# ubc-vision/COTR

Measured on NVIDIA H100. Metric: query-points/sec (256x256 pair, 1024 queries), higher is better.
Workload: dtype f32 (fp16 hi/lo split operands, fp32 accumulate on wgmma)

## Files before the change

### cotr_b200/csrc/mlp_tc.cu

```cuda
#include "split16.cuh"
#include "tc_common.cuh"

namespace cotr {

namespace {

using namespace tc;

constexpr int BM = 64;
constexpr int BK = 64;
constexpr int kThreads = 384;
constexpr int kConsumerThreads = 256;
constexpr int kBarConsumers = 6;
constexpr int kK1Chunks = kDModel / BK;

template <int S>
struct MlpCfg {
    static constexpr int HS = kFF / S;
    static constexpr int WN1 = HS / 2;
    static constexpr int kMain1 = WN1 >= 128 ? 1 : 2;
    static constexpr int kK2Chunks = HS / BK;
    static constexpr int kIters = kK1Chunks + kK2Chunks;
    static constexpr uint32_t kAPlane = BM * 128u;
    static constexpr uint32_t kW1Plane = HS * 128u;
    static constexpr uint32_t kW2Plane = kDModel * 128u;
    static constexpr uint32_t kStage1 = 2 * kAPlane + 2 * kW1Plane;
    static constexpr uint32_t kStage2 = 2 * kW2Plane;
    static constexpr uint32_t kStage = kStage1 > kStage2 ? kStage1 : kStage2;
    static constexpr uint32_t kHChunk = 2 * kAPlane;
    static constexpr uint32_t kHBytes = kK2Chunks * kHChunk;
    static constexpr int kStages = (int)((227u * 1024u - 2048u - kHBytes) / kStage);
    static constexpr uint32_t kHOffset = kStages * kStage;
    static constexpr uint32_t kBarOffset = kHOffset + kHBytes;
    static constexpr uint32_t kSmemBytes = kBarOffset + 256 + 1024;
    static constexpr uint32_t kAccPitch = kDModel * 4u + 16u;
    static constexpr uint32_t kAccBytes = ((BM * kAccPitch + 1023u) / 1024u) * 1024u;
    static constexpr int kOwnRows = BM / S;
    static constexpr uint32_t kRowBytes = kDModel * 4u;
    static constexpr uint32_t kPartOffset = kAccBytes;
    static constexpr uint32_t kPartBytes = (S - 1) * kOwnRows * kRowBytes;
    static_assert(kStages >= 2, "pipeline needs at least two stages");
    static_assert(kSmemBytes <= 227u * 1024u, "shared memory");
    static_assert(kPartOffset + kPartBytes <= kStages * kStage, "partial tiles do not fit the idle stages");
    static_assert(kStage % 1024 == 0 && kW1Plane % 1024 == 0 && kHBytes % 1024 == 0, "SWIZZLE_128B needs 1024-byte alignment");
};

template <int S>
__global__ void __launch_bounds__(kThreads, 1) mlp_tc_kernel(const MlpParams p) {
    using C = MlpCfg<S>;
    extern __shared__ uint8_t smem_raw[];
    const uint32_t raw_addr = smem_u32(smem_raw);
    uint8_t* base = smem_raw + (((raw_addr + 1023u) & ~1023u) - raw_addr);
    uint8_t* h_tile = base + C::kHOffset;
    uint64_t* full = reinterpret_cast<uint64_t*>(base + C::kBarOffset);
    uint64_t* empty = full + C::kStages;
    uint64_t* part_full = full + 2 * C::kStages;

    const int warp = threadIdx.x >> 5, lane = threadIdx.x & 31;
    const int rank = blockIdx.z;
    const int m0 = blockIdx.x * BM;
    const int h0 = rank * C::HS;

    if (threadIdx.x == 0) {
        for (int s = 0; s < C::kStages; ++s) {
            mbar_init(&full[s], 129);
            mbar_init(&empty[s], 8);
        }
        mbar_init(part_full, 1);
        mbar_fence_init();
        mbar_arrive_expect_tx(part_full, C::kPartBytes);
    }
    __syncthreads();

    if (warp >= 8) {
        const int t = threadIdx.x - kConsumerThreads;
        const int kg = t & 7;
        const int rb = t >> 3;
        const uint8_t* w1 = reinterpret_cast<const uint8_t*>(p.w1);
        const uint8_t* w2 = reinterpret_cast<const uint8_t*>(p.w2);
        auto load_weights = [&](int it) {
            const int s = it % C::kStages;
            uint8_t* dst = base + (size_t)s * C::kStage;
            if (it < kK1Chunks) {
                mbar_arrive_expect_tx(&full[s], 2u * C::kW1Plane);
                const uint8_t* src = w1 + ((size_t)(it * 2) * kFF + h0) * 128;
                tma_bulk_g2s(dst + 2 * C::kAPlane, src, C::kW1Plane, &full[s]);
                tma_bulk_g2s(dst + 2 * C::kAPlane + C::kW1Plane, src + (size_t)kFF * 128, C::kW1Plane, &full[s]);
            } else {
                mbar_arrive_expect_tx(&full[s], C::kStage2);
                tma_bulk_g2s(dst, w2 + (size_t)(h0 / BK + it - kK1Chunks) * C::kStage2, C::kStage2, &full[s]);
            }
        };
        if (t == 0) {
            for (int it = 0; it < C::kStages; ++it) load_weights(it);
            pdl_launch_dependents();
        }
        pdl_wait();
        const uint32_t a_off = (uint32_t)rb * 128u + (uint32_t)((kg ^ (rb & 7)) << 4);
#pragma unroll 1
        for (int it = 0; it < C::kIters; ++it) {
            const int s = it % C::kStages;
            const uint32_t ph = (uint32_t)(it / C::kStages) & 1u;
            mbar_wait(&empty[s], ph ^ 1u);
            if (t == 0 && it >= C::kStages) load_weights(it);
            if (it < kK1Chunks) {
                const uint32_t dst = smem_u32(base + (size_t)s * C::kStage) + a_off;
                const int k = it * BK + kg * 8;
#pragma unroll
                for (int i = 0; i < BM / 16; ++i) {
                    const int row = m0 + rb + 16 * i;
                    const bool ok = row < p.M;
                    const size_t off = ok ? (size_t)row * kDModel + k : 0;
                    cp_async16(dst + i * 2048, p.x.hi + off, ok ? 16u : 0u);
                    cp_async16(dst + C::kAPlane + i * 2048, p.x.lo + off, ok ? 16u : 0u);
                }
                cp_async_mbar_arrive_noinc(&full[s]);
            } else {
                mbar_arrive(&full[s]);
            }
        }
    } else {
        const int wg = warp >> 2;
        const int fr = (warp & 3) * 16 + (lane >> 2);
        const int fc = 2 * (lane & 3);
        {
            constexpr int WN = C::WN1, R = WN / 2;
            float acc_m[C::kMain1][R], acc_c[R];
#pragma unroll
            for (int a = 0; a < C::kMain1; ++a)
#pragma unroll
                for (int j = 0; j < R; ++j) acc_m[a][j] = 0.f;
#pragma unroll
            for (int j = 0; j < R; ++j) acc_c[j] = 0.f;
            auto mma = [&](float (&d)[R], uint64_t da, uint64_t db) {
                if constexpr (WN == 64) wgmma_ss_n64(d, da, db);
                else wgmma_ss_n128(d, da, db);
            };
            auto fence_all = [&]() {
#pragma unroll
                for (int a = 0; a < C::kMain1; ++a) fence_regs(acc_m[a]);
                fence_regs(acc_c);
            };
#pragma unroll 1
            for (int it = 0; it < kK1Chunks; ++it) {
                const int s = it % C::kStages;
                mbar_wait(&full[s], (uint32_t)(it / C::kStages) & 1u);
                fence_proxy_async_smem();
                const uint32_t a_addr = smem_u32(base + (size_t)s * C::kStage);
                const uint32_t b_addr = a_addr + 2 * C::kAPlane + (uint32_t)wg * WN * 128u;
                fence_all();
                wgmma_fence();
#pragma unroll
                for (int ks = 0; ks < BK / 16; ++ks) {
                    const uint64_t dah = make_desc_sw128(a_addr + 32 * ks);
                    const uint64_t dal = make_desc_sw128(a_addr + C::kAPlane + 32 * ks);
                    const uint64_t dbh = make_desc_sw128(b_addr + 32 * ks);
                    const uint64_t dbl = make_desc_sw128(b_addr + C::kW1Plane + 32 * ks);
                    mma(acc_c, dal, dbh);
                    mma(acc_m[ks % C::kMain1], dah, dbh);
                    mma(acc_c, dah, dbl);
                }
                wgmma_commit();
                wgmma_wait<1>();
                fence_all();
                if (it > 0 && lane == 0) mbar_arrive(&empty[(it - 1) % C::kStages]);
            }
            wgmma_wait<0>();
            fence_all();
            if (lane == 0) mbar_arrive(&empty[(kK1Chunks - 1) % C::kStages]);
#pragma unroll
            for (int j = 0; j < R; j += 2) {
                const int row = fr + ((j >> 1) & 1) * 8;
                const int c = wg * WN + (j >> 2) * 8 + fc;
                float v[2];
#pragma unroll
                for (int e = 0; e < 2; ++e) {
                    float y = acc_m[0][j + e];
#pragma unroll
                    for (int a = 1; a < C::kMain1; ++a) y += acc_m[a][j + e];
                    v[e] = fmaxf((acc_c[j + e] + y) * p.w1_scale + __ldg(p.b1 + h0 + c + e), 0.f);
                }
                uint32_t hi, lo;
                split_f16x2(v[0], v[1], hi, lo);
                const int cc = c & 63;
                uint8_t* d = h_tile + (uint32_t)(c >> 6) * C::kHChunk + (uint32_t)row * 128u + (uint32_t)((((cc >> 3) ^ (row & 7)) << 4) + (cc & 7) * 2);
                *reinterpret_cast<uint32_t*>(d) = hi;
                *reinterpret_cast<uint32_t*>(d + C::kAPlane) = lo;
            }
            fence_proxy_async_smem();
            named_barrier_sync(kBarConsumers, kConsumerThreads);
        }
        {
            float acc_m[64], acc_c[64];
#pragma unroll
            for (int j = 0; j < 64; ++j) { acc_m[j] = 0.f; acc_c[j] = 0.f; }
#pragma unroll 1
            for (int it = kK1Chunks; it < C::kIters; ++it) {
                const int s = it % C::kStages;
                mbar_wait(&full[s], (uint32_t)(it / C::kStages) & 1u);
                const uint32_t a_addr = smem_u32(h_tile) + (uint32_t)(it - kK1Chunks) * C::kHChunk;
                const uint32_t b_addr = smem_u32(base + (size_t)s * C::kStage) + (uint32_t)wg * 128u * 128u;
                fence_regs(acc_m);
                fence_regs(acc_c);
                wgmma_fence();
#pragma unroll
                for (int ks = 0; ks < BK / 16; ++ks) {
                    const uint64_t dah = make_desc_sw128(a_addr + 32 * ks);
                    const uint64_t dal = make_desc_sw128(a_addr + C::kAPlane + 32 * ks);
                    const uint64_t dbh = make_desc_sw128(b_addr + 32 * ks);
                    const uint64_t dbl = make_desc_sw128(b_addr + C::kW2Plane + 32 * ks);
                    wgmma_ss_n128(acc_c, dal, dbh);
                    wgmma_ss_n128(acc_m, dah, dbh);
                    wgmma_ss_n128(acc_c, dah, dbl);
                }
                wgmma_commit();
                wgmma_wait<1>();
                fence_regs(acc_m);
                fence_regs(acc_c);
                if (it > kK1Chunks && lane == 0) mbar_arrive(&empty[(it - 1) % C::kStages]);
            }
            wgmma_wait<0>();
            fence_regs(acc_m);
            fence_regs(acc_c);
            named_barrier_sync(kBarConsumers, kConsumerThreads);
#pragma unroll
            for (int j = 0; j < 64; j += 2) {
                const int row = fr + ((j >> 1) & 1) * 8;
                const int col = wg * 128 + (j >> 2) * 8 + fc;
                *reinterpret_cast<float2*>(base + (uint32_t)row * C::kAccPitch + col * 4) =
                    make_float2(acc_c[j] + acc_m[j], acc_c[j + 1] + acc_m[j + 1]);
            }
        }
    }

    __syncthreads();
    cluster_arrive();
    cluster_wait();
    {
        const uint32_t part_local = smem_u32(base) + C::kPartOffset;
        constexpr int kPieces = (BM - C::kOwnRows) * (C::kRowBytes / 16);
#pragma unroll 1
        for (int i = threadIdx.x; i < kPieces; i += kThreads) {
            const int pr = i / (C::kRowBytes / 16), piece = i % (C::kRowBytes / 16);
            const int r = pr < rank * C::kOwnRows ? pr : pr + C::kOwnRows;
            const int q = r / C::kOwnRows;
            const uint32_t slot = (uint32_t)(rank < q ? rank : rank - 1);
            const float4 v = *reinterpret_cast<const float4*>(base + (uint32_t)r * C::kAccPitch + piece * 16);
            const uint32_t dst = part_local + (slot * C::kOwnRows + (uint32_t)(r % C::kOwnRows)) * C::kRowBytes + piece * 16;
            st_async_f32x4(map_to_cta(dst, (uint32_t)q), v.x, v.y, v.z, v.w, map_to_cta(smem_u32(part_full), (uint32_t)q));
        }
    }
    if (warp < C::kOwnRows) mbar_wait(part_full, 0);
#pragma unroll 1
    for (int w = warp; w < C::kOwnRows; w += kThreads / 32) {
        const int rr = rank * C::kOwnRows + w;
        const int row = m0 + rr;
        if (row < p.M) {
            pdl_wait();
            float v[8];
            const uint8_t* own = base + (uint32_t)rr * C::kAccPitch + lane * 32;
            const float4 a0 = *reinterpret_cast<const float4*>(own), a1 = *reinterpret_cast<const float4*>(own + 16);
            v[0] = a0.x; v[1] = a0.y; v[2] = a0.z; v[3] = a0.w; v[4] = a1.x; v[5] = a1.y; v[6] = a1.z; v[7] = a1.w;
#pragma unroll 1
            for (int slot = 0; slot < S - 1; ++slot) {
                const uint8_t* pp = base + C::kPartOffset + (uint32_t)(slot * C::kOwnRows + w) * C::kRowBytes + lane * 32;
                const float4 b0 = *reinterpret_cast<const float4*>(pp), b1 = *reinterpret_cast<const float4*>(pp + 16);
                v[0] += b0.x; v[1] += b0.y; v[2] += b0.z; v[3] += b0.w; v[4] += b1.x; v[5] += b1.y; v[6] += b1.z; v[7] += b1.w;
            }
            float bias[8], res[8];
            load_vec8(p.b2, lane, bias);
            const size_t off = (size_t)row * kDModel + lane * 8;
            load8_split(p.x, off, res);
#pragma unroll
            for (int j = 0; j < 8; ++j) v[j] = v[j] * p.w2_scale + bias[j] + res[j];
            warp_layernorm256(v, p.g, p.be, lane);
            if (p.g2) warp_layernorm256(v, p.g2, p.be2, lane);
            store8_split(p.out, off, v);
        }
    }
}

template <int S>
int configure(size_t* smem) {
    static unsigned long long configured = 0;
    *smem = MlpCfg<S>::kSmemBytes;
    if (first_use_on_device(&configured))
        COTR_CHECK_CUDA(cudaFuncSetAttribute(mlp_tc_kernel<S>, cudaFuncAttributeMaxDynamicSharedMemorySize, (int)MlpCfg<S>::kSmemBytes));
    return 0;
}

int max_clusters_of_8(int* out) {
    static int cached[64] = {0};
    int dev = 0;
    cudaGetDevice(&dev);
    if (cached[dev & 63] > 0) { *out = cached[dev & 63]; return 0; }
    size_t smem = 0;
    if (configure<8>(&smem)) return 1;
    cudaLaunchConfig_t cfg = {};
    cfg.gridDim = dim3(1, 1, 8);
    cfg.blockDim = dim3(kThreads);
    cfg.dynamicSmemBytes = smem;
    cudaLaunchAttribute attr[1];
    attr[0].id = cudaLaunchAttributeClusterDimension;
    attr[0].val.clusterDim.x = 1;
    attr[0].val.clusterDim.y = 1;
    attr[0].val.clusterDim.z = 8;
    cfg.attrs = attr;
    cfg.numAttrs = 1;
    int n = 0;
    COTR_CHECK_CUDA(cudaOccupancyMaxActiveClusters(&n, mlp_tc_kernel<8>, &cfg));
    cached[dev & 63] = n;
    *out = n;
    return 0;
}

template <int S>
int launch_split(const MlpParams& p, cudaStream_t s) {
    size_t smem = 0;
    if (configure<S>(&smem)) return 1;
    const dim3 grid((p.M + BM - 1) / BM, 1, S);
    COTR_CHECK_CUDA(launch_kernel_cluster(mlp_tc_kernel<S>, grid, dim3(kThreads), smem, s, S, p));
    return 0;
}

}

int launch_mlp_tc(const MlpParams& p, cudaStream_t s) {
    COTR_CHECK(p.M > 0 && p.w1 && p.w2 && p.b1 && p.b2 && p.g && p.be && (p.g2 == nullptr) == (p.be2 == nullptr),
               "mlp_tc: bad parameters (M %d)", p.M);
    const int tiles = (p.M + BM - 1) / BM;
    int n8 = 0;
    if (max_clusters_of_8(&n8)) return 1;
    return launch_mlp_tc_split(p, tiles <= n8 ? 8 : 4, s);
}

int launch_mlp_tc_split(const MlpParams& p, int S, cudaStream_t s) {
    COTR_CHECK(S == 4 || S == 8, "mlp_tc: hidden split %d (4 or 8)", S);
    return S == 8 ? launch_split<8>(p, s) : launch_split<4>(p, s);
}

}
```

### cotr_b200/csrc/tc_common.cuh

```cuda
#pragma once
#include <cuda_fp16.h>
#include <cuda_runtime.h>
#include <cstdint>

namespace cotr {
namespace tc {

__device__ __forceinline__ uint32_t smem_u32(const void* p) {
    return static_cast<uint32_t>(__cvta_generic_to_shared(p));
}

__device__ __forceinline__ void mbar_init(uint64_t* bar, uint32_t count) {
    asm volatile("mbarrier.init.shared::cta.b64 [%0], %1;" ::"r"(smem_u32(bar)), "r"(count) : "memory");
}
__device__ __forceinline__ void mbar_fence_init() {
    asm volatile("fence.mbarrier_init.release.cluster;" ::: "memory");
}
__device__ __forceinline__ void mbar_arrive(uint64_t* bar) {
    asm volatile("mbarrier.arrive.shared::cta.b64 _, [%0];" ::"r"(smem_u32(bar)) : "memory");
}
__device__ __forceinline__ void mbar_arrive_expect_tx(uint64_t* bar, uint32_t bytes) {
    asm volatile("mbarrier.arrive.expect_tx.shared::cta.b64 _, [%0], %1;" ::"r"(smem_u32(bar)), "r"(bytes) : "memory");
}
__device__ __forceinline__ bool mbar_try_wait(uint64_t* bar, uint32_t parity) {
    uint32_t ok;
    asm volatile(
        "{\n\t.reg .pred p;\n\t"
        "mbarrier.try_wait.parity.shared::cta.b64 p, [%1], %2;\n\t"
        "selp.u32 %0, 1, 0, p;\n\t}"
        : "=r"(ok)
        : "r"(smem_u32(bar)), "r"(parity)
        : "memory");
    return ok != 0;
}
__device__ __forceinline__ void mbar_wait(uint64_t* bar, uint32_t parity) {
    while (!mbar_try_wait(bar, parity)) {
    }
}

__device__ __forceinline__ void fence_proxy_async_smem() {
    asm volatile("fence.proxy.async.shared::cta;" ::: "memory");
}

__device__ __forceinline__ void ld_cg_32b(const void* p, uint4& a, uint4& b) {
    a = __ldcg(reinterpret_cast<const uint4*>(p));
    b = __ldcg(reinterpret_cast<const uint4*>(p) + 1);
}

__device__ __forceinline__ void cp_async16(uint32_t smem_dst, const void* gmem_src, uint32_t src_bytes) {
    asm volatile("cp.async.cg.shared.global [%0], [%1], 16, %2;" ::"r"(smem_dst), "l"(gmem_src), "r"(src_bytes) : "memory");
}
__device__ __forceinline__ void cp_async_mbar_arrive_noinc(uint64_t* bar) {
    asm volatile("cp.async.mbarrier.arrive.noinc.shared::cta.b64 [%0];" ::"r"(smem_u32(bar)) : "memory");
}

__device__ __forceinline__ void named_barrier_sync(int id, int threads) {
    asm volatile("bar.sync %0, %1;" ::"r"(id), "r"(threads) : "memory");
}

__device__ __forceinline__ void named_barrier_arrive(int id, int threads) {
    asm volatile("bar.arrive %0, %1;" ::"r"(id), "r"(threads) : "memory");
}

__device__ __forceinline__ void cluster_arrive() { asm volatile("barrier.cluster.arrive.release;" ::: "memory"); }
__device__ __forceinline__ void cluster_wait() { asm volatile("barrier.cluster.wait.acquire;" ::: "memory"); }
__device__ __forceinline__ uint32_t map_to_cta(uint32_t smem_addr, uint32_t rank) {
    uint32_t r;
    asm volatile("mapa.shared::cluster.u32 %0, %1, %2;" : "=r"(r) : "r"(smem_addr), "r"(rank));
    return r;
}
__device__ __forceinline__ void st_cluster_f32x4(uint32_t cluster_addr, float a, float b, float c, float d) {
    asm volatile("st.shared::cluster.v4.f32 [%0], {%1, %2, %3, %4};" ::"r"(cluster_addr), "f"(a), "f"(b), "f"(c), "f"(d) : "memory");
}

__device__ __forceinline__ void st_async_f32x4(uint32_t cluster_addr, float a, float b, float c, float d, uint32_t cluster_mbar) {
    asm volatile("st.async.weak.shared::cluster.mbarrier::complete_tx::bytes.v4.f32 [%0], {%1, %2, %3, %4}, [%5];"
                 ::"r"(cluster_addr), "f"(a), "f"(b), "f"(c), "f"(d), "r"(cluster_mbar)
                 : "memory");
}
__device__ __forceinline__ void cluster_arrive_relaxed() { asm volatile("barrier.cluster.arrive.relaxed;" ::: "memory"); }

__device__ __forceinline__ void tma_bulk_g2s(void* smem_dst, const void* gmem_src, uint32_t bytes, uint64_t* bar) {
    asm volatile("cp.async.bulk.shared::cluster.global.mbarrier::complete_tx::bytes [%0], [%1], %2, [%3];"
                 ::"r"(smem_u32(smem_dst)), "l"(gmem_src), "r"(bytes), "r"(smem_u32(bar))
                 : "memory");
}

__device__ __forceinline__ uint64_t make_smem_desc(uint32_t smem_addr, uint32_t lbo_bytes, uint32_t sbo_bytes) {
    const uint32_t lo = ((smem_addr & 0x3FFFFu) >> 4) | (((lbo_bytes >> 4) & 0x3FFFu) << 16);
    const uint32_t hi = (sbo_bytes >> 4) & 0x3FFFu;
    return (uint64_t)lo | ((uint64_t)hi << 32);
}
__device__ __forceinline__ uint64_t make_desc_sw128(uint32_t smem_addr) {
    const uint32_t lo = ((smem_addr & 0x3FFFFu) >> 4) | (1u << 16);
    const uint32_t hi = (1024u >> 4) | (1u << 30);
    return (uint64_t)lo | ((uint64_t)hi << 32);
}

__device__ __forceinline__ void wgmma_fence() { asm volatile("wgmma.fence.sync.aligned;" ::: "memory"); }
__device__ __forceinline__ void wgmma_commit() { asm volatile("wgmma.commit_group.sync.aligned;" ::: "memory"); }
template <int N>
__device__ __forceinline__ void wgmma_wait() { asm volatile("wgmma.wait_group.sync.aligned %0;" ::"n"(N) : "memory"); }
template <int R>
__device__ __forceinline__ void fence_regs(float (&d)[R]) {
#pragma unroll
    for (int i = 0; i < R; ++i) asm volatile("" : "+f"(d[i])::"memory");
}

__device__ __forceinline__ void wgmma_ss_n16(float (&d)[8], uint64_t a_desc, uint64_t b_desc) {
    asm volatile(
        "wgmma.mma_async.sync.aligned.m64n16k16.f32.f16.f16 {%0,%1,%2,%3,%4,%5,%6,%7}, %8, %9, 1, 1, 1, 0, 0;"
        : "+f"(d[0]), "+f"(d[1]), "+f"(d[2]), "+f"(d[3]), "+f"(d[4]), "+f"(d[5]), "+f"(d[6]), "+f"(d[7])
        : "l"(a_desc), "l"(b_desc));
}
__device__ __forceinline__ void wgmma_ss_n32(float (&d)[16], uint64_t a_desc, uint64_t b_desc) {
    asm volatile(
        "wgmma.mma_async.sync.aligned.m64n32k16.f32.f16.f16 {%0,%1,%2,%3,%4,%5,%6,%7,%8,%9,%10,%11,%12,%13,%14,%15}, %16, %17, 1, 1, 1, 0, 0;"
        : "+f"(d[0]), "+f"(d[1]), "+f"(d[2]), "+f"(d[3]), "+f"(d[4]), "+f"(d[5]), "+f"(d[6]), "+f"(d[7]), "+f"(d[8]), "+f"(d[9]), "+f"(d[10]), "+f"(d[11]), "+f"(d[12]), "+f"(d[13]), "+f"(d[14]), "+f"(d[15])
        : "l"(a_desc), "l"(b_desc));
}
__device__ __forceinline__ void wgmma_ss_n64(float (&d)[32], uint64_t a_desc, uint64_t b_desc) {
    asm volatile(
        "wgmma.mma_async.sync.aligned.m64n64k16.f32.f16.f16 {%0,%1,%2,%3,%4,%5,%6,%7,%8,%9,%10,%11,%12,%13,%14,%15,%16,%17,%18,%19,%20,%21,%22,%23,%24,%25,%26,%27,%28,%29,%30,%31}, %32, %33, 1, 1, 1, 0, 0;"
        : "+f"(d[0]), "+f"(d[1]), "+f"(d[2]), "+f"(d[3]), "+f"(d[4]), "+f"(d[5]), "+f"(d[6]), "+f"(d[7]), "+f"(d[8]), "+f"(d[9]), "+f"(d[10]), "+f"(d[11]), "+f"(d[12]), "+f"(d[13]), "+f"(d[14]), "+f"(d[15]), "+f"(d[16]), "+f"(d[17]), "+f"(d[18]), "+f"(d[19]), "+f"(d[20]), "+f"(d[21]), "+f"(d[22]), "+f"(d[23]), "+f"(d[24]), "+f"(d[25]), "+f"(d[26]), "+f"(d[27]), "+f"(d[28]), "+f"(d[29]), "+f"(d[30]), "+f"(d[31])
        : "l"(a_desc), "l"(b_desc));
}
__device__ __forceinline__ void wgmma_ss_n128(float (&d)[64], uint64_t a_desc, uint64_t b_desc) {
    asm volatile(
        "wgmma.mma_async.sync.aligned.m64n128k16.f32.f16.f16 {%0,%1,%2,%3,%4,%5,%6,%7,%8,%9,%10,%11,%12,%13,%14,%15,%16,%17,%18,%19,%20,%21,%22,%23,%24,%25,%26,%27,%28,%29,%30,%31,%32,%33,%34,%35,%36,%37,%38,%39,%40,%41,%42,%43,%44,%45,%46,%47,%48,%49,%50,%51,%52,%53,%54,%55,%56,%57,%58,%59,%60,%61,%62,%63}, %64, %65, 1, 1, 1, 0, 0;"
        : "+f"(d[0]), "+f"(d[1]), "+f"(d[2]), "+f"(d[3]), "+f"(d[4]), "+f"(d[5]), "+f"(d[6]), "+f"(d[7]), "+f"(d[8]), "+f"(d[9]), "+f"(d[10]), "+f"(d[11]), "+f"(d[12]), "+f"(d[13]), "+f"(d[14]), "+f"(d[15]), "+f"(d[16]), "+f"(d[17]), "+f"(d[18]), "+f"(d[19]), "+f"(d[20]), "+f"(d[21]), "+f"(d[22]), "+f"(d[23]), "+f"(d[24]), "+f"(d[25]), "+f"(d[26]), "+f"(d[27]), "+f"(d[28]), "+f"(d[29]), "+f"(d[30]), "+f"(d[31]), "+f"(d[32]), "+f"(d[33]), "+f"(d[34]), "+f"(d[35]), "+f"(d[36]), "+f"(d[37]), "+f"(d[38]), "+f"(d[39]), "+f"(d[40]), "+f"(d[41]), "+f"(d[42]), "+f"(d[43]), "+f"(d[44]), "+f"(d[45]), "+f"(d[46]), "+f"(d[47]), "+f"(d[48]), "+f"(d[49]), "+f"(d[50]), "+f"(d[51]), "+f"(d[52]), "+f"(d[53]), "+f"(d[54]), "+f"(d[55]), "+f"(d[56]), "+f"(d[57]), "+f"(d[58]), "+f"(d[59]), "+f"(d[60]), "+f"(d[61]), "+f"(d[62]), "+f"(d[63])
        : "l"(a_desc), "l"(b_desc));
}
__device__ __forceinline__ void wgmma_rs_n32(float (&d)[16], const uint32_t (&a)[4], uint64_t b_desc) {
    asm volatile(
        "wgmma.mma_async.sync.aligned.m64n32k16.f32.f16.f16 {%0,%1,%2,%3,%4,%5,%6,%7,%8,%9,%10,%11,%12,%13,%14,%15}, {%16,%17,%18,%19}, %20, 1, 1, 1, 0;"
        : "+f"(d[0]), "+f"(d[1]), "+f"(d[2]), "+f"(d[3]), "+f"(d[4]), "+f"(d[5]), "+f"(d[6]), "+f"(d[7]), "+f"(d[8]), "+f"(d[9]), "+f"(d[10]), "+f"(d[11]), "+f"(d[12]), "+f"(d[13]), "+f"(d[14]), "+f"(d[15])
        : "r"(a[0]), "r"(a[1]), "r"(a[2]), "r"(a[3]), "l"(b_desc));
}

}
}
```

Baseline: 1.063 million.

## Fuse hi/lo weight wgmmas into single n256 instruction via interleaved B layout

```diff
diff --git a/cotr_b200/csrc/mlp_tc.cu b/cotr_b200/csrc/mlp_tc.cu
--- a/cotr_b200/csrc/mlp_tc.cu
+++ b/cotr_b200/csrc/mlp_tc.cu
@@ -84,11 +84,15 @@
             if (it < kK1Chunks) {
                 mbar_arrive_expect_tx(&full[s], 2u * C::kW1Plane);
                 const uint8_t* src = w1 + ((size_t)(it * 2) * kFF + h0) * 128;
-                tma_bulk_g2s(dst + 2 * C::kAPlane, src, C::kW1Plane, &full[s]);
-                tma_bulk_g2s(dst + 2 * C::kAPlane + C::kW1Plane, src + (size_t)kFF * 128, C::kW1Plane, &full[s]);
+                for (int q = 0; q < 4; ++q)
+                    tma_bulk_g2s(dst + 2 * C::kAPlane + q * C::kW1Plane / 2,
+                                 src + (size_t)(~q & 1) * kFF * 128 + (q >> 1) * C::kW1Plane / 2, C::kW1Plane / 2, &full[s]);
             } else {
                 mbar_arrive_expect_tx(&full[s], C::kStage2);
-                tma_bulk_g2s(dst, w2 + (size_t)(h0 / BK + it - kK1Chunks) * C::kStage2, C::kStage2, &full[s]);
+                const uint8_t* src = w2 + (size_t)(h0 / BK + it - kK1Chunks) * C::kStage2;
+                for (int q = 0; q < 4; ++q)
+                    tma_bulk_g2s(dst + q * C::kW2Plane / 2, src + (~q & 1) * C::kW2Plane + (q >> 1) * C::kW2Plane / 2,
+                                 C::kW2Plane / 2, &full[s]);
             }
         };
         if (t == 0) {
@@ -147,18 +151,22 @@
                 mbar_wait(&full[s], (uint32_t)(it / C::kStages) & 1u);
                 fence_proxy_async_smem();
                 const uint32_t a_addr = smem_u32(base + (size_t)s * C::kStage);
-                const uint32_t b_addr = a_addr + 2 * C::kAPlane + (uint32_t)wg * WN * 128u;
+                const uint32_t b_addr = a_addr + 2 * C::kAPlane + (uint32_t)wg * 2u * WN * 128u;
                 fence_all();
                 wgmma_fence();
 #pragma unroll
                 for (int ks = 0; ks < BK / 16; ++ks) {
                     const uint64_t dah = make_desc_sw128(a_addr + 32 * ks);
                     const uint64_t dal = make_desc_sw128(a_addr + C::kAPlane + 32 * ks);
-                    const uint64_t dbh = make_desc_sw128(b_addr + 32 * ks);
-                    const uint64_t dbl = make_desc_sw128(b_addr + C::kW1Plane + 32 * ks);
+                    const uint64_t dbl = make_desc_sw128(b_addr + 32 * ks);
+                    const uint64_t dbh = make_desc_sw128(b_addr + WN * 128u + 32 * ks);
                     mma(acc_c, dal, dbh);
-                    mma(acc_m[ks % C::kMain1], dah, dbh);
-                    mma(acc_c, dah, dbl);
+                    if constexpr (C::kMain1 == 1) {
+                        wgmma_ss_n256_pair(acc_c, acc_m[0], dah, dbl);
+                    } else {
+                        mma(acc_m[ks % C::kMain1], dah, dbh);
+                        mma(acc_c, dah, dbl);
+                    }
                 }
                 wgmma_commit();
                 wgmma_wait<1>();
@@ -199,7 +207,7 @@
                 const int s = it % C::kStages;
                 mbar_wait(&full[s], (uint32_t)(it / C::kStages) & 1u);
                 const uint32_t a_addr = smem_u32(h_tile) + (uint32_t)(it - kK1Chunks) * C::kHChunk;
-                const uint32_t b_addr = smem_u32(base + (size_t)s * C::kStage) + (uint32_t)wg * 128u * 128u;
+                const uint32_t b_addr = smem_u32(base + (size_t)s * C::kStage) + (uint32_t)wg * C::kW2Plane;
                 fence_regs(acc_m);
                 fence_regs(acc_c);
                 wgmma_fence();
@@ -207,11 +215,10 @@
                 for (int ks = 0; ks < BK / 16; ++ks) {
                     const uint64_t dah = make_desc_sw128(a_addr + 32 * ks);
                     const uint64_t dal = make_desc_sw128(a_addr + C::kAPlane + 32 * ks);
-                    const uint64_t dbh = make_desc_sw128(b_addr + 32 * ks);
-                    const uint64_t dbl = make_desc_sw128(b_addr + C::kW2Plane + 32 * ks);
+                    const uint64_t dbl = make_desc_sw128(b_addr + 32 * ks);
+                    const uint64_t dbh = make_desc_sw128(b_addr + 128u * 128u + 32 * ks);
                     wgmma_ss_n128(acc_c, dal, dbh);
-                    wgmma_ss_n128(acc_m, dah, dbh);
-                    wgmma_ss_n128(acc_c, dah, dbl);
+                    wgmma_ss_n256_pair(acc_c, acc_m, dah, dbl);
                 }
                 wgmma_commit();
                 wgmma_wait<1>();
diff --git a/cotr_b200/csrc/tc_common.cuh b/cotr_b200/csrc/tc_common.cuh
--- a/cotr_b200/csrc/tc_common.cuh
+++ b/cotr_b200/csrc/tc_common.cuh
@@ -137,6 +137,12 @@
         : "+f"(d[0]), "+f"(d[1]), "+f"(d[2]), "+f"(d[3]), "+f"(d[4]), "+f"(d[5]), "+f"(d[6]), "+f"(d[7]), "+f"(d[8]), "+f"(d[9]), "+f"(d[10]), "+f"(d[11]), "+f"(d[12]), "+f"(d[13]), "+f"(d[14]), "+f"(d[15])
         : "r"(a[0]), "r"(a[1]), "r"(a[2]), "r"(a[3]), "l"(b_desc));
 }
+__device__ __forceinline__ void wgmma_ss_n256_pair(float (&d)[64], float (&e)[64], uint64_t a_desc, uint64_t b_desc) {
+    asm volatile(
+        "wgmma.mma_async.sync.aligned.m64n256k16.f32.f16.f16 {%0,%1,%2,%3,%4,%5,%6,%7,%8,%9,%10,%11,%12,%13,%14,%15,%16,%17,%18,%19,%20,%21,%22,%23,%24,%25,%26,%27,%28,%29,%30,%31,%32,%33,%34,%35,%36,%37,%38,%39,%40,%41,%42,%43,%44,%45,%46,%47,%48,%49,%50,%51,%52,%53,%54,%55,%56,%57,%58,%59,%60,%61,%62,%63,%64,%65,%66,%67,%68,%69,%70,%71,%72,%73,%74,%75,%76,%77,%78,%79,%80,%81,%82,%83,%84,%85,%86,%87,%88,%89,%90,%91,%92,%93,%94,%95,%96,%97,%98,%99,%100,%101,%102,%103,%104,%105,%106,%107,%108,%109,%110,%111,%112,%113,%114,%115,%116,%117,%118,%119,%120,%121,%122,%123,%124,%125,%126,%127}, %128, %129, 1, 1, 1, 0, 0;"
+        : "+f"(d[0]), "+f"(d[1]), "+f"(d[2]), "+f"(d[3]), "+f"(d[4]), "+f"(d[5]), "+f"(d[6]), "+f"(d[7]), "+f"(d[8]), "+f"(d[9]), "+f"(d[10]), "+f"(d[11]), "+f"(d[12]), "+f"(d[13]), "+f"(d[14]), "+f"(d[15]), "+f"(d[16]), "+f"(d[17]), "+f"(d[18]), "+f"(d[19]), "+f"(d[20]), "+f"(d[21]), "+f"(d[22]), "+f"(d[23]), "+f"(d[24]), "+f"(d[25]), "+f"(d[26]), "+f"(d[27]), "+f"(d[28]), "+f"(d[29]), "+f"(d[30]), "+f"(d[31]), "+f"(d[32]), "+f"(d[33]), "+f"(d[34]), "+f"(d[35]), "+f"(d[36]), "+f"(d[37]), "+f"(d[38]), "+f"(d[39]), "+f"(d[40]), "+f"(d[41]), "+f"(d[42]), "+f"(d[43]), "+f"(d[44]), "+f"(d[45]), "+f"(d[46]), "+f"(d[47]), "+f"(d[48]), "+f"(d[49]), "+f"(d[50]), "+f"(d[51]), "+f"(d[52]), "+f"(d[53]), "+f"(d[54]), "+f"(d[55]), "+f"(d[56]), "+f"(d[57]), "+f"(d[58]), "+f"(d[59]), "+f"(d[60]), "+f"(d[61]), "+f"(d[62]), "+f"(d[63]), "+f"(e[0]), "+f"(e[1]), "+f"(e[2]), "+f"(e[3]), "+f"(e[4]), "+f"(e[5]), "+f"(e[6]), "+f"(e[7]), "+f"(e[8]), "+f"(e[9]), "+f"(e[10]), "+f"(e[11]), "+f"(e[12]), "+f"(e[13]), "+f"(e[14]), "+f"(e[15]), "+f"(e[16]), "+f"(e[17]), "+f"(e[18]), "+f"(e[19]), "+f"(e[20]), "+f"(e[21]), "+f"(e[22]), "+f"(e[23]), "+f"(e[24]), "+f"(e[25]), "+f"(e[26]), "+f"(e[27]), "+f"(e[28]), "+f"(e[29]), "+f"(e[30]), "+f"(e[31]), "+f"(e[32]), "+f"(e[33]), "+f"(e[34]), "+f"(e[35]), "+f"(e[36]), "+f"(e[37]), "+f"(e[38]), "+f"(e[39]), "+f"(e[40]), "+f"(e[41]), "+f"(e[42]), "+f"(e[43]), "+f"(e[44]), "+f"(e[45]), "+f"(e[46]), "+f"(e[47]), "+f"(e[48]), "+f"(e[49]), "+f"(e[50]), "+f"(e[51]), "+f"(e[52]), "+f"(e[53]), "+f"(e[54]), "+f"(e[55]), "+f"(e[56]), "+f"(e[57]), "+f"(e[58]), "+f"(e[59]), "+f"(e[60]), "+f"(e[61]), "+f"(e[62]), "+f"(e[63])
+        : "l"(a_desc), "l"(b_desc));
+}
 
 }
 }
```

Result: no change. 1.066 million, median of 6 (+0.3%).
